# facebookresearch/pytorchvideo

Hardware: AMD Instinct MI355X
Metric: clips/sec forward (higher is better)
Workload: dtype bf16; 1 GPU; x3d_m: create_x3d(input_clip_length=16,input_crop_size=224) [B,3,16,224,224]; per_gpu_batch=32, global_batch=32, parallelism=dp1 (batch-sharded, logits all_gather), head_collective=none (one rank: the logits stay where they are), hip_graph=True, streams=2

## Files before the change

pytorchvideo_amd/csrc/pv_conv.hip:

```cpp
#include "pv_common.h"

#include <stdlib.h>
int pv_pwconv_stream_try(const pv_conv3d_desc& d, hipStream_t s);
int pv_gemm_glds_try(const pv_conv3d_desc& d, bool pw, hipStream_t s);
int pv_head_rows_try(const pv_conv3d_desc& d, hipStream_t s);
int pv_gemm8_try(const pv_conv3d_desc& d, bool pw, hipStream_t s);
int pv_gemm9_try(const pv_conv3d_desc& d, bool pw, hipStream_t s);
int pv_tapstream_try(const pv_conv3d_desc& d, hipStream_t s, bool dry = false);
int pv_stem_c4(const pv_conv3d_desc& d, hipStream_t s);
int pv_stem_dwt_supported(const pv_conv3d_desc& d);
int pv_stem_ncdhw_supported(const pv_conv3d_desc& d);
int pv_pwconv_x2_supported(const pv_conv3d_desc& d);

namespace {

constexpr int kThreads = 256;
constexpr int kBK = 32;
constexpr int kMaxTaps = 512;

template <typename T> struct LdsLd { static constexpr int v = kBK + 8; };
template <> struct LdsLd<float> { static constexpr int v = kBK + 4; };

template <typename T, int BM, int BN, int WM_, int WN_, bool PW>
__global__ __launch_bounds__(kThreads) void conv_igemm_kernel(const pv_conv3d_desc d) {
  constexpr int LD = LdsLd<T>::v;
  constexpr int TM = BM / WM_ / 16;
  constexpr int TN = BN / WN_ / 16;
  static_assert(WM_ * WN_ == 4, "4 waves");
  static_assert(TN % 2 == 0, "channel tiles are stored in pairs");
  constexpr int KC = kBK / 8;
  constexpr int XCH = BM * KC / kThreads;
  constexpr int WCH = (BN * KC + kThreads - 1) / kThreads;
  static_assert(BM * KC % kThreads == 0, "");

  __shared__ __attribute__((aligned(16))) T smem[2 * (BM + BN) * LD];
  __shared__ int s_tap[PW ? 1 : kMaxTaps];
  constexpr int kGateMaxC = 512;
  __shared__ __attribute__((aligned(16))) float s_gate[PW ? 2 * kGateMaxC : 4];

  const int tid = threadIdx.x;
  const int lane = tid & 63;
  const int wave = tid >> 6;
  const int wm = wave % WM_;
  const int wn = wave / WM_;
  const int l15 = lane & 15;
  const int q = lane >> 4;

  const int S_out = d.To * d.Ho * d.Wo;
  const long M = (long)d.B * S_out;
  const int taps = d.kt * d.kh * d.kw;
  const int K = taps * d.cin;
  const int cout_p8 = pv_round_up(d.cout, 8);
  const int n_tiles_n = (cout_p8 + BN - 1) / BN;
  const int tile_n = blockIdx.x % n_tiles_n;
  const long tile_m = blockIdx.x / n_tiles_n;
  const long m0 = tile_m * BM;
  const int n0 = tile_n * BN;

  const T* __restrict__ X = static_cast<const T*>(d.x);
  const T* __restrict__ Wt = static_cast<const T*>(d.w);

  if constexpr (!PW) {
    for (int t = tid; t < taps; t += kThreads) {
      const int dt = t / (d.kh * d.kw);
      const int r = t - dt * d.kh * d.kw;
      const int dh = r / d.kw;
      const int dw = r - dh * d.kw;
      s_tap[t] = (dt * (d.dil_t > 1 ? d.dil_t : 1)) | ((dh * (d.dil_h > 1 ? d.dil_h : 1)) << 8) |
                 ((dw * (d.dil_w > 1 ? d.dil_w : 1)) << 16);
    }
    __syncthreads();
  }

  bool gate_lds = false;
  int gate_b0 = 0;
  if constexpr (PW) {
    if (d.a_gate != nullptr) {
      gate_b0 = (int)(m0 / S_out);
      const long m_last = (m0 + BM < M ? m0 + BM : M) - 1;
      gate_lds = d.cin <= kGateMaxC && (d.cin & 7) == 0 && (int)(m_last / S_out) - gate_b0 <= 1;
      if (gate_lds) {
        const float* __restrict__ base = d.a_gate + (long)gate_b0 * d.cin;
        const int n_ok = gate_b0 + 1 < d.B ? 2 * d.cin : d.cin;
        constexpr int GT = 2 * kGateMaxC / kThreads;
        float gv[GT];
#pragma unroll
        for (int k = 0; k < GT; ++k) {
          const int i = tid + k * kThreads;
          gv[k] = base[i < n_ok ? i : 0];
        }
        pv_wait_loads();
#pragma unroll
        for (int k = 0; k < GT; ++k) {
          const int i = tid + k * kThreads;
          if (i < 2 * d.cin) s_gate[i] = i < n_ok ? gv[k] : 0.f;
        }
        __syncthreads();
      }
    }
  }

  const int kc = tid % KC;
  long x_off[XCH];
  int x_t[XCH], x_h[XCH], x_w[XCH];
  int x_b[XCH];
  bool x_ok[XCH];
#pragma unroll
  for (int i = 0; i < XCH; ++i) {
    const int r = tid / KC + i * (kThreads / KC);
    const long m = m0 + r;
    x_ok[i] = m < M;
    const long mm = x_ok[i] ? m : 0;
    const int b = (int)(mm / S_out);
    const int sp = (int)(mm - (long)b * S_out);
    x_b[i] = b;
    if constexpr (PW) {
      x_off[i] = (long)b * d.x_bs + (long)sp * d.ldx;
      x_t[i] = x_h[i] = x_w[i] = 0;
    } else {
      const int to = sp / (d.Ho * d.Wo);
      const int r2 = sp - to * d.Ho * d.Wo;
      const int ho = r2 / d.Wo;
      const int wo = r2 - ho * d.Wo;
      x_off[i] = (long)b * d.x_bs;
      x_t[i] = to * d.st - d.pt;
      x_h[i] = ho * d.sh - d.ph;
      x_w[i] = wo * d.sw - d.pw;
    }
  }
  int w_row[WCH];
  long w_off[WCH];
  bool w_ok[WCH];
#pragma unroll
  for (int i = 0; i < WCH; ++i) {
    const int id = tid + i * kThreads;
    const int r = id / KC;
    w_row[i] = r;
    const int wv = r / (TN * 16);
    const int rr = r - wv * (TN * 16);
    const int tn = rr >> 4;
    const int ii = rr & 15;
    const int c = n0 + wv * (TN * 16) + (tn >> 1) * 32 + (ii >> 2) * 8 + (tn & 1) * 4 + (ii & 3);
    w_ok[i] = (id < BN * KC) && (c < d.cout);
    w_off[i] = (long)c * K;
  }

  Chunk8<T> xrA[XCH], wrA[WCH], xrB[XCH], wrB[WCH];

  auto load_global = [&](Chunk8<T> (&xr)[XCH], Chunk8<T> (&wr)[WCH], int ks) {
    const int k0 = ks * kBK + kc * 8;
    if constexpr (PW) {
      const bool kok = k0 < K;
#pragma unroll
      for (int i = 0; i < XCH; ++i) {
        if (x_ok[i] && kok) xr[i].load(X + x_off[i] + k0);
        else xr[i].zero();
      }
    } else {
      const int tap = k0 / d.cin;
      const int c = k0 - tap * d.cin;
      const bool kok = tap < taps;
      const int tp = kok ? s_tap[tap] : 0;
      const int dt = tp & 255, dh = (tp >> 8) & 255, dw = tp >> 16;
#pragma unroll
      for (int i = 0; i < XCH; ++i) {
        const int ti = x_t[i] + dt, hi = x_h[i] + dh, wi = x_w[i] + dw;
        const bool ok = x_ok[i] && kok && (unsigned)ti < (unsigned)d.Ti &&
                        (unsigned)hi < (unsigned)d.Hi && (unsigned)wi < (unsigned)d.Wi;
        if (ok) xr[i].load(X + x_off[i] + ((long)(ti * d.Hi + hi) * d.Wi + wi) * d.ldx + c);
        else xr[i].zero();
      }
    }
#pragma unroll
    for (int i = 0; i < WCH; ++i) {
      if (w_ok[i] && k0 < K) wr[i].load(Wt + w_off[i] + k0);
      else wr[i].zero();
    }
  };

  auto store_lds = [&](Chunk8<T> (&xr)[XCH], Chunk8<T> (&wr)[WCH], int buf, int ks) {
    T* xs = smem + buf * (BM + BN) * LD;
    T* ws = xs + BM * LD;
    const int k0 = ks * kBK + kc * 8;
#pragma unroll
    for (int i = 0; i < XCH; ++i) {
      const int r = tid / KC + i * (kThreads / KC);
      if (d.a_gate != nullptr || d.a_act != PV_ACT_NONE) {
        float f[8];
        xr[i].to_f32(f);
        if (d.a_gate != nullptr && k0 < K) {
          float4 g0, g1;
          if (PW && gate_lds) {
            const float* g = s_gate + (x_ok[i] ? x_b[i] - gate_b0 : 0) * d.cin + k0;
            g0 = *reinterpret_cast<const float4*>(g);
            g1 = *reinterpret_cast<const float4*>(g + 4);
          } else {
            const float* g = d.a_gate + (long)x_b[i] * d.cin + k0;
            g0 = *reinterpret_cast<const float4*>(g);
            g1 = *reinterpret_cast<const float4*>(g + 4);
          }
          f[0] *= g0.x; f[1] *= g0.y; f[2] *= g0.z; f[3] *= g0.w;
          f[4] *= g1.x; f[5] *= g1.y; f[6] *= g1.z; f[7] *= g1.w;
        }
        pv_apply_act_n<sizeof(T) == 2>(f, d.a_act);
        xr[i].from_f32(f);
      }
      xr[i].store(xs + r * LD + kc * 8);
    }
#pragma unroll
    for (int i = 0; i < WCH; ++i) {
      const int id = tid + i * kThreads;
      if (id < BN * KC) wr[i].store(ws + w_row[i] * LD + kc * 8);
    }
  };

  f32x4 acc[TN][TM];
#pragma unroll
  for (int a = 0; a < TN; ++a)
#pragma unroll
    for (int b = 0; b < TM; ++b) acc[a][b] = f32x4{0.f, 0.f, 0.f, 0.f};

  const int wave_c0 = n0 + wn * (TN * 16);

  const int nk = (K + kBK - 1) / kBK;
  auto compute = [&](int buf) {
    const T* xs = smem + buf * (BM + BN) * LD;
    const T* ws = xs + BM * LD;
    if constexpr (sizeof(T) == 2) {
      bf16x8 xf[TM], wf[TN];
#pragma unroll
      for (int t = 0; t < TM; ++t)
        xf[t] = *reinterpret_cast<const bf16x8*>(xs + (wm * TM * 16 + t * 16 + l15) * LD + q * 8);
#pragma unroll
      for (int t = 0; t < TN; ++t)
        wf[t] = *reinterpret_cast<const bf16x8*>(ws + (wn * TN * 16 + t * 16 + l15) * LD + q * 8);
#pragma unroll
      for (int a = 0; a < TN; ++a) {
        if (wave_c0 + (a >> 1) * 32 < cout_p8) {
#pragma unroll
          for (int b = 0; b < TM; ++b)
            acc[a][b] = __builtin_amdgcn_mfma_f32_16x16x32_bf16(wf[a], xf[b], acc[a][b], 0, 0, 0);
        }
      }
    } else {
#pragma unroll
      for (int kk = 0; kk < kBK / 4; ++kk) {
        float xf[TM], wf[TN];
#pragma unroll
        for (int t = 0; t < TM; ++t) xf[t] = (float)xs[(wm * TM * 16 + t * 16 + l15) * LD + kk * 4 + q];
#pragma unroll
        for (int t = 0; t < TN; ++t) wf[t] = (float)ws[(wn * TN * 16 + t * 16 + l15) * LD + kk * 4 + q];
#pragma unroll
        for (int a = 0; a < TN; ++a) {
          if (wave_c0 + (a >> 1) * 32 < cout_p8) {
#pragma unroll
            for (int b = 0; b < TM; ++b)
              acc[a][b] = __builtin_amdgcn_mfma_f32_16x16x4f32(wf[a], xf[b], acc[a][b], 0, 0, 0);
          }
        }
      }
    }
  };
  load_global(xrA, wrA, 0);
  store_lds(xrA, wrA, 0, 0);
  if (nk > 1) load_global(xrA, wrA, 1);
  if (nk > 2) load_global(xrB, wrB, 2);
  __syncthreads();
  for (int ks = 0; ks < nk; ks += 2) {
    compute(0);
    if (ks + 1 < nk) store_lds(xrA, wrA, 1, ks + 1);
    if (ks + 3 < nk) load_global(xrA, wrA, ks + 3);
    __syncthreads();
    if (ks + 1 >= nk) break;
    compute(1);
    if (ks + 2 < nk) store_lds(xrB, wrB, 0, ks + 2);
    if (ks + 4 < nk) load_global(xrB, wrB, ks + 4);
    __syncthreads();
  }

  const T* __restrict__ R = static_cast<const T*>(d.residual);
#pragma unroll
  for (int p = 0; p < TN / 2; ++p) {
    const int c0 = wave_c0 + p * 32 + q * 8;
    if (c0 >= cout_p8) continue;
    float sc[8], sh[8];
#pragma unroll
    for (int j = 0; j < 8; ++j) {
      const bool ok = (c0 + j) < d.cout;
      sc[j] = ok ? (d.scale ? d.scale[c0 + j] : 1.0f) : 0.0f;
      sh[j] = ok ? (d.shift ? d.shift[c0 + j] : 0.0f) : 0.0f;
    }
#pragma unroll
    for (int t = 0; t < TM; ++t) {
      const long m = m0 + wm * (TM * 16) + t * 16 + l15;
      if (m >= M) continue;
      const int b = (int)(m / S_out);
      const long sp = m - (long)b * S_out;
      float v[8];
#pragma unroll
      for (int j = 0; j < 4; ++j) {
        v[j] = acc[2 * p][t][j] * sc[j] + sh[j];
        v[4 + j] = acc[2 * p + 1][t][j] * sc[4 + j] + sh[4 + j];
      }
      if (R != nullptr) {
        float rf[8];
        if (d.r_f32) {
          Chunk8<float> rc;
          rc.load(static_cast<const float*>(d.residual) + (long)b * d.r_bs + sp * d.ldr + c0);
          rc.to_f32(rf);
        } else {
          Chunk8<T> rc;
          rc.load(R + (long)b * d.r_bs + sp * d.ldr + c0);
          rc.to_f32(rf);
        }
#pragma unroll
        for (int j = 0; j < 8; ++j) v[j] += rf[j];
      }
      pv_apply_act_n<sizeof(T) == 2>(v, d.act);
#pragma unroll
      for (int j = 0; j < 8; ++j)
        if (c0 + j >= d.cout) v[j] = 0.0f;
      const long yo = (long)b * d.y_bs + sp * d.ldy + c0;
      if (d.y_f32) {
        Chunk8<float> oc;
        oc.from_f32(v);
        oc.store(static_cast<float*>(d.y) + yo);
      } else {
        Chunk8<T> oc;
        oc.from_f32(v);
        oc.store(static_cast<T*>(d.y) + yo);
      }
    }
  }
}

template <typename T, int BM, int BN, int WM_, int WN_>
int launch_cfg(const pv_conv3d_desc& d, bool pw, hipStream_t s) {
  const long M = (long)d.B * d.To * d.Ho * d.Wo;
  const int cout_p8 = pv_round_up(d.cout, 8);
  const long tiles = pv_ceil_div(M, BM) * pv_ceil_div(cout_p8, BN);
  if (tiles <= 0 || tiles > 0x7fffffffL) return PV_ERR_INVALID;
  dim3 grid((unsigned)tiles), block(kThreads);
  if (pw) PV_LAUNCH((conv_igemm_kernel<T, BM, BN, WM_, WN_, true>), grid, block, 0, s, d);
  else PV_LAUNCH((conv_igemm_kernel<T, BM, BN, WM_, WN_, false>), grid, block, 0, s, d);
  PV_LAUNCH_CHECK();
  return PV_OK;
}

template <typename T> int launch_conv(const pv_conv3d_desc& d, bool pw, hipStream_t s) {
  const int cout_p8 = pv_round_up(d.cout, 8);
  if (cout_p8 <= 32) return launch_cfg<T, 256, 32, 4, 1>(d, pw, s);
  if (cout_p8 <= 64) return launch_cfg<T, 128, 64, 4, 1>(d, pw, s);
  return launch_cfg<T, 128, 128, 2, 2>(d, pw, s);
}

}

extern "C" int pv_conv3d_dwt_supported(const pv_conv3d_desc* d) {
  if (!d || d->B <= 0 || d->cout <= 0 || d->To <= 0 || d->Ho <= 0 || d->Wo <= 0) return 0;
  return pv_stem_dwt_supported(*d);
}

extern "C" int pv_conv3d_ncdhw_supported(const pv_conv3d_desc* d) {
  if (!d || d->B <= 0 || d->cout <= 0 || d->To <= 0 || d->Ho <= 0 || d->Wo <= 0 || d->Ti <= 0 || d->Hi <= 0 || d->Wi <= 0) return 0;
  return pv_stem_ncdhw_supported(*d);
}

extern "C" int pv_conv3d_pw2_supported(const pv_conv3d_desc* d) {
  if (!d || d->B <= 0 || d->cin <= 0 || d->cout <= 0 || d->pw2_cout <= 0 || d->To <= 0 || d->Ho <= 0 || d->Wo <= 0) return 0;
  if (d->kt < 1 || d->kh < 1 || d->kw < 1 || d->kt * d->kh * d->kw == 1) return 0;
  return pv_tapstream_try(*d, nullptr, true) == PV_OK;
}

extern "C" int pv_conv3d_x2_supported(const pv_conv3d_desc* d) {
  if (!d || d->B <= 0 || d->cout <= 0 || d->To <= 0 || d->Ho <= 0 || d->Wo <= 0) return 0;
  if (d->kt * d->kh * d->kw != 1 || d->st != 1 || d->sh != 1 || d->sw != 1 || d->pt || d->ph || d->pw) return 0;
  return pv_pwconv_x2_supported(*d);
}

extern "C" int pv_conv3d(const pv_conv3d_desc* dp, pv_stream_t stream) {
  if (!dp) return PV_ERR_INVALID;
  const pv_conv3d_desc& d = *dp;
  if (!d.x || !d.w || !d.y) return PV_ERR_INVALID;
  if (d.B <= 0 || d.cin <= 0 || d.cout <= 0 || d.To <= 0 || d.Ho <= 0 || d.Wo <= 0) return PV_ERR_INVALID;
  const bool c4 = d.cin == 4 && d.ldx == 4 && d.dtype == PV_BF16;
  if (!c4 && (d.cin % 8 || d.ldx % 8 || d.x_bs % 8)) return PV_ERR_INVALID;
  if (d.ldy % 8 || d.y_bs % 8 || (c4 && d.x_bs % 4)) return PV_ERR_INVALID;
  if (d.residual && (d.ldr % 8 || d.r_bs % 8)) return PV_ERR_INVALID;
  if (d.kt < 1 || d.kh < 1 || d.kw < 1 || d.st < 1 || d.sh < 1 || d.sw < 1) return PV_ERR_INVALID;
  const int taps = d.kt * d.kh * d.kw;
  if (taps > kMaxTaps || d.kt > 255 || d.kh > 255 || d.kw > 255) return PV_ERR_UNSUPPORTED;
  if (d.dil_t < 0 || d.dil_h < 0 || d.dil_w < 0) return PV_ERR_INVALID;
  const int et = (d.kt - 1) * (d.dil_t > 1 ? d.dil_t : 1) + 1, eh = (d.kh - 1) * (d.dil_h > 1 ? d.dil_h : 1) + 1,
            ew = (d.kw - 1) * (d.dil_w > 1 ? d.dil_w : 1) + 1;
  if (et > 255 || eh > 255 || ew > 255) return PV_ERR_UNSUPPORTED;
  const bool dilated = et != d.kt || eh != d.kh || ew != d.kw;
  if (dilated && c4) return PV_ERR_UNSUPPORTED;
  if ((d.Ti + 2 * d.pt - et) / d.st + 1 != d.To || (d.Hi + 2 * d.ph - eh) / d.sh + 1 != d.Ho ||
      (d.Wi + 2 * d.pw - ew) / d.sw + 1 != d.Wo)
    return PV_ERR_INVALID;
  const bool pw = taps == 1 && d.st == 1 && d.sh == 1 && d.sw == 1 && d.pt == 0 && d.ph == 0 && d.pw == 0;
  if ((d.a_gate || d.a_act != PV_ACT_NONE) && !pw) return PV_ERR_UNSUPPORTED;
  hipStream_t s = static_cast<hipStream_t>(stream);
  if (c4) return pv_stem_c4(d, s);
  if (d.dwt_w || d.pos_spatial || d.pos_temporal) return PV_ERR_UNSUPPORTED;
  if (d.pw2_w) {
    if (pw || d.x2 || d.pw2_cout <= 0 || d.dtype != PV_BF16) return PV_ERR_UNSUPPORTED;
    return pv_tapstream_try(d, s);
  }
  if (d.x2) {
    if (!pw || d.dtype != PV_BF16 || !pv_pwconv_x2_supported(d)) return PV_ERR_UNSUPPORTED;
    return pv_pwconv_stream_try(d, s);
  }
  if (d.dtype == PV_BF16) {
    const int route = pv_tune("conv_route", 0);
    const int cout_p8 = pv_round_up(d.cout, 8);
    const int small_cin = pv_tune("conv_small_cin", 128);
    const bool small = d.cin <= small_cin;
    if (route != 3) {
      if (pw && route == 0 && pv_tune("head_rows", 1)) {
        const int r = pv_head_rows_try(d, s);
        if (r != PV_ERR_UNSUPPORTED) return r;
      }
      if (pw && (route == 1 || (route == 0 && small))) {
        const int r = pv_pwconv_stream_try(d, s);
        if (r != PV_ERR_UNSUPPORTED) return r;
      }
      if (!pw && cout_p8 <= 64 && (long)taps * d.cin <= 640 && pv_tune("tapstream_first", 1)) {
        const int r = pv_tapstream_try(d, s);
        if (r != PV_ERR_UNSUPPORTED) return r;
      }
      const bool gemm_ok = route == 2 || pw || (cout_p8 >= 64 && d.cin >= 64);
      int r = gemm_ok ? pv_gemm9_try(d, pw, s) : PV_ERR_UNSUPPORTED;
      if (r != PV_ERR_UNSUPPORTED) return r;
      r = gemm_ok ? pv_gemm8_try(d, pw, s) : PV_ERR_UNSUPPORTED;
      if (r != PV_ERR_UNSUPPORTED) return r;
      r = gemm_ok ? pv_gemm_glds_try(d, pw, s) : PV_ERR_UNSUPPORTED;
      if (r != PV_ERR_UNSUPPORTED) return r;
      if (pw) {
        r = pv_pwconv_stream_try(d, s);
        if (r != PV_ERR_UNSUPPORTED) return r;
      }
    }
  }
  if (d.dtype == PV_BF16 && !pw) {
    const int r = pv_tapstream_try(d, s);
    if (r != PV_ERR_UNSUPPORTED) return r;
  }
  if (d.dtype == PV_BF16) return launch_conv<bf16_t>(d, pw, s);
  if (d.dtype == PV_F32) return launch_conv<float>(d, pw, s);
  return PV_ERR_UNSUPPORTED;
}
```

Baseline: 11850 clips/s.

## Use buffer-resource loads and specialized gate/swish paths in pointwise igemm

Adds templated variants of the pointwise bf16 implicit-GEMM kernel that load activations and weights through raw buffer loads. These rely on hardware out-of-bounds zeroing instead of per-chunk bounds branches. A gate+swish specialization prefetches the SE gate into LDS alongside the first tile, and the main loop is restructured to drop per-iteration tail checks. A tune knob for forcing BN=64 tiles is also added. The changes add template instantiations and code size, and rely on the descriptor bounds fitting in 32-bit buffer ranges.

```diff
diff --git a/pytorchvideo_amd/csrc/pv_conv.hip b/pytorchvideo_amd/csrc/pv_conv.hip
--- a/pytorchvideo_amd/csrc/pv_conv.hip
+++ b/pytorchvideo_amd/csrc/pv_conv.hip
@@ -17,13 +17,18 @@
 constexpr int kThreads = 256;
 constexpr int kBK = 32;
 constexpr int kMaxTaps = 512;
+constexpr int kGateMaxC = 512;
 
 template <typename T> struct LdsLd { static constexpr int v = kBK + 8; };
 template <> struct LdsLd<float> { static constexpr int v = kBK + 4; };
 
-template <typename T, int BM, int BN, int WM_, int WN_, bool PW>
+enum { kFxOff = 0, kFxPlain = 1, kFxGateSwish = 2, kFxAny = 3 };
+
+template <typename T, int BM, int BN, int WM_, int WN_, bool PW, int FX = kFxOff>
 __global__ __launch_bounds__(kThreads) void conv_igemm_kernel(const pv_conv3d_desc d) {
   constexpr int LD = LdsLd<T>::v;
+  constexpr bool BUF = FX != kFxOff;
+  static_assert(!BUF || (PW && sizeof(T) == 2), "buffer-addressed operands: pointwise bf16 only");
   constexpr int TM = BM / WM_ / 16;
   constexpr int TN = BN / WN_ / 16;
   static_assert(WM_ * WN_ == 4, "4 waves");
@@ -35,7 +40,6 @@
 
   __shared__ __attribute__((aligned(16))) T smem[2 * (BM + BN) * LD];
   __shared__ int s_tap[PW ? 1 : kMaxTaps];
-  constexpr int kGateMaxC = 512;
   __shared__ __attribute__((aligned(16))) float s_gate[PW ? 2 * kGateMaxC : 4];
 
   const int tid = threadIdx.x;
@@ -74,7 +78,20 @@
 
   bool gate_lds = false;
   int gate_b0 = 0;
-  if constexpr (PW) {
+  const int gate_pitch = pv_round_up(d.cin, kBK);
+  constexpr int GT = 2 * kGateMaxC / kThreads;
+  float gv[GT];
+  if constexpr (FX == kFxGateSwish) {
+    gate_b0 = (int)(m0 / S_out);
+    const float* __restrict__ base = d.a_gate + (long)gate_b0 * d.cin;
+    const bool has_next = gate_b0 + 1 < d.B;
+#pragma unroll
+    for (int k = 0; k < GT; ++k) {
+      const int i = tid + k * kThreads;
+      const int r = i >= gate_pitch ? 1 : 0, c = i - r * gate_pitch;
+      gv[k] = base[c < d.cin && (r == 0 || has_next) ? r * d.cin + c : 0];
+    }
+  } else if constexpr (PW && FX != kFxPlain) {
     if (d.a_gate != nullptr) {
       gate_b0 = (int)(m0 / S_out);
       const long m_last = (m0 + BM < M ? m0 + BM : M) - 1;
@@ -144,11 +161,38 @@
     w_ok[i] = (id < BN * KC) && (c < d.cout);
     w_off[i] = (long)c * K;
   }
+  constexpr unsigned kOob = 0x80000000u;
+  __amdgpu_buffer_rsrc_t rx, rw;
+  unsigned x_bo[XCH], w_bo[WCH];
+  int g_lo[XCH];
+  if constexpr (BUF) {
+    const long x_elems = (long)(d.B - 1) * d.x_bs + (long)(S_out - 1) * d.ldx + d.cin;
+    rx = __builtin_amdgcn_make_buffer_rsrc(const_cast<T*>(X), 0, (int)(x_elems * 2), 0x00020000);
+    rw = __builtin_amdgcn_make_buffer_rsrc(const_cast<T*>(Wt), 0, (int)((long)d.cout * K * 2), 0x00020000);
+#pragma unroll
+    for (int i = 0; i < XCH; ++i) {
+      x_bo[i] = x_ok[i] ? (unsigned)(x_off[i] * 2) + (unsigned)kc * 16u : kOob;
+      g_lo[i] = (x_ok[i] ? x_b[i] - gate_b0 : 0) * gate_pitch + kc * 8;
+    }
+#pragma unroll
+    for (int i = 0; i < WCH; ++i) w_bo[i] = w_ok[i] ? (unsigned)(w_off[i] * 2) + (unsigned)kc * 16u : kOob;
+  }
 
   Chunk8<T> xrA[XCH], wrA[WCH], xrB[XCH], wrB[WCH];
 
   auto load_global = [&](Chunk8<T> (&xr)[XCH], Chunk8<T> (&wr)[WCH], int ks) {
     const int k0 = ks * kBK + kc * 8;
+    if constexpr (BUF) {
+      const unsigned kb = (unsigned)ks * (kBK * 2);
+      const bool kok = k0 < K;
+#pragma unroll
+      for (int i = 0; i < XCH; ++i)
+        xr[i].v = __builtin_bit_cast(bf16x8, __builtin_amdgcn_raw_buffer_load_b128(rx, (int)(kok ? x_bo[i] + kb : kOob), 0, 0));
+#pragma unroll
+      for (int i = 0; i < WCH; ++i)
+        wr[i].v = __builtin_bit_cast(bf16x8, __builtin_amdgcn_raw_buffer_load_b128(rw, (int)(kok ? w_bo[i] + kb : kOob), 0, 0));
+      return;
+    }
     if constexpr (PW) {
       const bool kok = k0 < K;
 #pragma unroll
@@ -185,7 +229,19 @@
 #pragma unroll
     for (int i = 0; i < XCH; ++i) {
       const int r = tid / KC + i * (kThreads / KC);
-      if (d.a_gate != nullptr || d.a_act != PV_ACT_NONE) {
+      if constexpr (FX == kFxGateSwish) {
+        float f[8];
+        xr[i].to_f32(f);
+        const float* g = s_gate + g_lo[i] + ks * kBK;
+        const float4 g0 = *reinterpret_cast<const float4*>(g);
+        const float4 g1 = *reinterpret_cast<const float4*>(g + 4);
+        f[0] *= g0.x; f[1] *= g0.y; f[2] *= g0.z; f[3] *= g0.w;
+        f[4] *= g1.x; f[5] *= g1.y; f[6] *= g1.z; f[7] *= g1.w;
+#pragma unroll
+        for (int j = 0; j < 8; ++j) f[j] *= pv_sigmoid(f[j]);
+        xr[i].from_f32(f);
+      } else if constexpr (FX == kFxPlain) {
+      } else if (d.a_gate != nullptr || d.a_act != PV_ACT_NONE) {
         float f[8];
         xr[i].to_f32(f);
         if (d.a_gate != nullptr && k0 < K) {
@@ -210,7 +266,7 @@
 #pragma unroll
     for (int i = 0; i < WCH; ++i) {
       const int id = tid + i * kThreads;
-      if (id < BN * KC) wr[i].store(ws + w_row[i] * LD + kc * 8);
+      if ((BUF && BN * KC % kThreads == 0) || id < BN * KC) wr[i].store(ws + w_row[i] * LD + kc * 8);
     }
   };
 
@@ -220,7 +276,7 @@
 #pragma unroll
     for (int b = 0; b < TM; ++b) acc[a][b] = f32x4{0.f, 0.f, 0.f, 0.f};
 
-  const int wave_c0 = n0 + wn * (TN * 16);
+  const int wave_c0 = n0 + (BUF ? __builtin_amdgcn_readfirstlane(wn) : wn) * (TN * 16);
 
   const int nk = (K + kBK - 1) / kBK;
   auto compute = [&](int buf) {
@@ -261,21 +317,57 @@
       }
     }
   };
-  load_global(xrA, wrA, 0);
-  store_lds(xrA, wrA, 0, 0);
-  if (nk > 1) load_global(xrA, wrA, 1);
-  if (nk > 2) load_global(xrB, wrB, 2);
-  __syncthreads();
-  for (int ks = 0; ks < nk; ks += 2) {
+  if constexpr (BUF) {
+    load_global(xrA, wrA, 0);
+    if constexpr (FX == kFxGateSwish) {
+      const bool has_next = gate_b0 + 1 < d.B;
+      pv_wait_loads();
+#pragma unroll
+      for (int k = 0; k < GT; ++k) {
+        const int i = tid + k * kThreads;
+        const int r = i >= gate_pitch ? 1 : 0, c = i - r * gate_pitch;
+        if (i < 2 * gate_pitch) s_gate[i] = c >= d.cin ? 1.0f : (r == 0 || has_next) ? gv[k] : 0.f;
+      }
+      __syncthreads();
+    }
+    store_lds(xrA, wrA, 0, 0);
+    load_global(xrA, wrA, 1);
+    load_global(xrB, wrB, 2);
+    __syncthreads();
+    int ks = 0;
+    for (; ks + 2 < nk; ks += 2) {
+      compute(0);
+      store_lds(xrA, wrA, 1, ks + 1);
+      load_global(xrA, wrA, ks + 3);
+      __syncthreads();
+      compute(1);
+      store_lds(xrB, wrB, 0, ks + 2);
+      load_global(xrB, wrB, ks + 4);
+      __syncthreads();
+    }
     compute(0);
-    if (ks + 1 < nk) store_lds(xrA, wrA, 1, ks + 1);
-    if (ks + 3 < nk) load_global(xrA, wrA, ks + 3);
+    if (ks + 1 < nk) {
+      store_lds(xrA, wrA, 1, ks + 1);
+      __syncthreads();
+      compute(1);
+    }
+  } else {
+    load_global(xrA, wrA, 0);
+    store_lds(xrA, wrA, 0, 0);
+    if (nk > 1) load_global(xrA, wrA, 1);
+    if (nk > 2) load_global(xrB, wrB, 2);
     __syncthreads();
-    if (ks + 1 >= nk) break;
-    compute(1);
-    if (ks + 2 < nk) store_lds(xrB, wrB, 0, ks + 2);
-    if (ks + 4 < nk) load_global(xrB, wrB, ks + 4);
-    __syncthreads();
+    for (int ks = 0; ks < nk; ks += 2) {
+      compute(0);
+      if (ks + 1 < nk) store_lds(xrA, wrA, 1, ks + 1);
+      if (ks + 3 < nk) load_global(xrA, wrA, ks + 3);
+      __syncthreads();
+      if (ks + 1 >= nk) break;
+      compute(1);
+      if (ks + 2 < nk) store_lds(xrB, wrB, 0, ks + 2);
+      if (ks + 4 < nk) load_global(xrB, wrB, ks + 4);
+      __syncthreads();
+    }
   }
 
   const T* __restrict__ R = static_cast<const T*>(d.residual);
@@ -334,6 +426,20 @@
   }
 }
 
+int pw_operand_path(const pv_conv3d_desc& d, int bm) {
+  if (!pv_tune("igemm_pw_buf", 1)) return kFxOff;
+  const long S_out = (long)d.To * d.Ho * d.Wo, M = (long)d.B * S_out;
+  if (d.x_bs < 0 || d.ldx < d.cin) return kFxOff;
+  const long x_bytes = ((long)(d.B - 1) * d.x_bs + (S_out - 1) * d.ldx + d.cin) * 2, w_bytes = (long)d.cout * d.cin * 2;
+  if (x_bytes > 0x7fffffffL || w_bytes > 0x7fffffffL) return kFxOff;
+  if (!d.a_gate && d.a_act == PV_ACT_NONE) return kFxPlain;
+  if (!d.a_gate || d.a_act != PV_ACT_SWISH || d.cin > kGateMaxC) return kFxAny;
+  if (S_out < bm - 1)
+    for (long m0 = 0; m0 < M; m0 += bm)
+      if (((m0 + bm < M ? m0 + bm : M) - 1) / S_out - m0 / S_out > 1) return kFxAny;
+  return kFxGateSwish;
+}
+
 template <typename T, int BM, int BN, int WM_, int WN_>
 int launch_cfg(const pv_conv3d_desc& d, bool pw, hipStream_t s) {
   const long M = (long)d.B * d.To * d.Ho * d.Wo;
@@ -341,6 +447,14 @@
   const long tiles = pv_ceil_div(M, BM) * pv_ceil_div(cout_p8, BN);
   if (tiles <= 0 || tiles > 0x7fffffffL) return PV_ERR_INVALID;
   dim3 grid((unsigned)tiles), block(kThreads);
+  if constexpr (sizeof(T) == 2) {
+    switch (pw ? pw_operand_path(d, BM) : kFxOff) {
+      case kFxPlain: PV_LAUNCH((conv_igemm_kernel<T, BM, BN, WM_, WN_, true, kFxPlain>), grid, block, 0, s, d); PV_LAUNCH_CHECK(); return PV_OK;
+      case kFxGateSwish: PV_LAUNCH((conv_igemm_kernel<T, BM, BN, WM_, WN_, true, kFxGateSwish>), grid, block, 0, s, d); PV_LAUNCH_CHECK(); return PV_OK;
+      case kFxAny: PV_LAUNCH((conv_igemm_kernel<T, BM, BN, WM_, WN_, true, kFxAny>), grid, block, 0, s, d); PV_LAUNCH_CHECK(); return PV_OK;
+      default: break;
+    }
+  }
   if (pw) PV_LAUNCH((conv_igemm_kernel<T, BM, BN, WM_, WN_, true>), grid, block, 0, s, d);
   else PV_LAUNCH((conv_igemm_kernel<T, BM, BN, WM_, WN_, false>), grid, block, 0, s, d);
   PV_LAUNCH_CHECK();
@@ -350,7 +464,7 @@
 template <typename T> int launch_conv(const pv_conv3d_desc& d, bool pw, hipStream_t s) {
   const int cout_p8 = pv_round_up(d.cout, 8);
   if (cout_p8 <= 32) return launch_cfg<T, 256, 32, 4, 1>(d, pw, s);
-  if (cout_p8 <= 64) return launch_cfg<T, 128, 64, 4, 1>(d, pw, s);
+  if (cout_p8 <= 64 || pv_tune("igemm_bn64", 0)) return launch_cfg<T, 128, 64, 4, 1>(d, pw, s);
   return launch_cfg<T, 128, 128, 2, 2>(d, pw, s);
 }
 
```

Result: faster. 11970 clips/s (median of 6 runs) (+1.0%).
